# volume-em/empanada-napari

Measured on AMD Instinct MI355X. Metric: EM tiles/sec (1024^2 fp16), higher is better.
Workload: dtype f16

## Files before the change

### empanada-napari_amd/csrc/conv3x3c64.hip

```cpp
#include "igemm_common.h"

namespace emp {
namespace {

constexpr int C64_TH = 8, C64_TW = 16;
constexpr int C64_IH = C64_TH + 2, C64_IW = C64_TW + 2;
constexpr int C64_NPIX = C64_IH * C64_IW;
constexpr int C64_NPC = (C64_NPIX + 7) / 8;
constexpr int C64_SLOT = (C64_NPC + 1) * 1024;
constexpr int C64_NDMA = 3;

struct C64Params {
  const half_t* in;
  const half_t* wgt;
  const float* bias;
  half_t* out;
  const half_t* zero;
  int N, H, W, in_ld, out_ld, act;
  int tiles_x, tiles_y, tiles;
};

template <int ACT>
__global__ void __launch_bounds__(512, 1) conv3x3_c64_kernel(const C64Params p) {
  extern __shared__ __attribute__((aligned(1024))) char lds[];
  const int tid = threadIdx.x, lane = tid & 63;
  const int wave = __builtin_amdgcn_readfirstlane(tid >> 6);
  const int pg = wave >> 1, ch = wave & 1;
  const int fr = lane & 15, fq = lane >> 4;

  const int xcd = blockIdx.x & 7, jx = blockIdx.x >> 3, nx = gridDim.x >> 3;
  auto tile_of = [&](int it) { return (it * 8 + xcd) * nx + jx; };
  int my_tiles = 0;
  while (tile_of(my_tiles) < p.tiles) ++my_tiles;

  f16x8 wreg[2][9][2];
#pragma unroll
  for (int c = 0; c < 2; ++c) {
    const half_t* wr = p.wgt + (size_t)(ch * 32 + perm32(c * 16 + fr)) * (9 * 64) + fq * 8;
#pragma unroll
    for (int t = 0; t < 9; ++t)
#pragma unroll
      for (int kk = 0; kk < 2; ++kk) wreg[c][t][kk] = *reinterpret_cast<const f16x8*>(wr + t * 64 + kk * 32);
  }
  float bv[8];
  {
    const int co = ch * 32 + fq * 8;
#pragma unroll
    for (int r = 0; r < 8; ++r) bv[r] = p.bias ? p.bias[co + r] : 0.f;
  }
  asm volatile("s_waitcnt vmcnt(0)" ::: "memory");

  auto stage = [&](int it, int slot) {
    const bool valid = it < my_tiles;
    int n = 0, y0 = 0, x0 = 0;
    if (valid) {
      const int tile = tile_of(it);
      const int tx = tile % p.tiles_x, r = tile / p.tiles_x;
      const int ty = r % p.tiles_y;
      n = r / p.tiles_y;
      y0 = ty * C64_TH;
      x0 = tx * C64_TW;
    }
    char* hb = lds + slot * C64_SLOT;
#pragma unroll
    for (int k = 0; k < C64_NDMA; ++k) {
      const int piece = wave + 8 * k;
      const int hp = piece * 8 + (lane >> 3);
      const int hy = hp / C64_IW, hx = hp - hy * C64_IW;
      const int iy = y0 + hy - 1, ix = x0 + hx - 1;
      const bool ok = valid && wave + 8 * k < C64_NPC && hp < C64_NPIX && (unsigned)iy < (unsigned)p.H &&
                      (unsigned)ix < (unsigned)p.W;
      const half_t* src = ok ? p.in + (((size_t)n * p.H + iy) * p.W + ix) * p.in_ld + (((lane & 7) ^ (hp & 7)) << 3)
                             : p.zero;
      lds_dma16(src, hb + piece * 1024);
    }
  };

  stage(0, 0);
  stage(1, 1);
  asm volatile("s_waitcnt vmcnt(3)" ::: "memory");
  lds_barrier();

  int slot = 0;
  for (int it = 0; it < my_tiles; ++it) {
    stage(it + 2, slot == 0 ? 2 : slot - 1);
    const char* hb = lds + slot * C64_SLOT;
    f32x4 acc[2][2];
#pragma unroll
    for (int c = 0; c < 2; ++c)
#pragma unroll
      for (int t = 0; t < 2; ++t) acc[c][t] = f32x4{0.f, 0.f, 0.f, 0.f};
#pragma unroll
    for (int tap = 0; tap < 9; ++tap) {
      const int dy = tap / 3, dx = tap - dy * 3;
#pragma unroll
      for (int kk = 0; kk < 2; ++kk) {
        f16x8 pf[2];
#pragma unroll
        for (int t = 0; t < 2; ++t) {
          const int hp = (2 * pg + t + dy) * C64_IW + fr + dx;
          pf[t] = *reinterpret_cast<const f16x8*>(hb + hp * 128 + (((kk * 4 + fq) ^ (hp & 7)) << 4));
        }
#pragma unroll
        for (int c = 0; c < 2; ++c)
#pragma unroll
          for (int t = 0; t < 2; ++t)
            acc[c][t] = __builtin_amdgcn_mfma_f32_16x16x32_f16(wreg[c][tap][kk], pf[t], acc[c][t], 0, 0, 0);
      }
    }
    asm volatile("s_waitcnt vmcnt(3)" ::: "memory");
    {
      const int tile = tile_of(it);
      const int tx = tile % p.tiles_x, r = tile / p.tiles_x;
      const int ty = r % p.tiles_y, n = r / p.tiles_y;
      const int ox = tx * C64_TW + fr;
#pragma unroll
      for (int t = 0; t < 2; ++t) {
        const int oy = ty * C64_TH + 2 * pg + t;
        f16x8 o;
#pragma unroll
        for (int r4 = 0; r4 < 4; ++r4) {
          o[r4] = (half_t)conv_act<ACT>(acc[0][t][r4] + bv[r4]);
          o[4 + r4] = (half_t)conv_act<ACT>(acc[1][t][r4] + bv[4 + r4]);
        }
        if (oy < p.H && ox < p.W)
          *reinterpret_cast<f16x8*>(p.out + (((size_t)n * p.H + oy) * p.W + ox) * p.out_ld + ch * 32 + fq * 8) = o;
      }
    }
    lds_barrier();
    slot = slot == 2 ? 0 : slot + 1;
  }
  asm volatile("s_waitcnt vmcnt(0)" ::: "memory");
}

constexpr int C128_NDMA = 6;
constexpr int C128_SLOT = 8 * C128_NDMA * 1024;

template <int ACT>
__global__ void __launch_bounds__(512, 1) conv3x3_c128_kernel(const C64Params p) {
  extern __shared__ __attribute__((aligned(1024))) char lds[];
  const int tid = threadIdx.x, lane = tid & 63;
  const int wave = __builtin_amdgcn_readfirstlane(tid >> 6);
  const int fr = lane & 15, fq = lane >> 4;
  const int xcd = blockIdx.x & 7, jx = blockIdx.x >> 3, nx = gridDim.x >> 3;
  auto tile_of = [&](int it) { return (it * 8 + xcd) * nx + jx; };
  int my_tiles = 0;
  while (tile_of(my_tiles) < p.tiles) ++my_tiles;

  f16x8 wreg[9][4];
  {
    const half_t* wr = p.wgt + (size_t)(16 * wave + fr) * (9 * 128) + fq * 8;
#pragma unroll
    for (int t = 0; t < 9; ++t)
#pragma unroll
      for (int kk = 0; kk < 4; ++kk) wreg[t][kk] = *reinterpret_cast<const f16x8*>(wr + t * 128 + kk * 32);
  }
  float bv[4];
#pragma unroll
  for (int r = 0; r < 4; ++r) bv[r] = p.bias ? p.bias[16 * wave + fq * 4 + r] : 0.f;
  asm volatile("s_waitcnt vmcnt(0)" ::: "memory");

  auto tile_xy = [&](int it, int& n, int& y0, int& x0) {
    const int tile = tile_of(it);
    const int tx = tile % p.tiles_x, r = tile / p.tiles_x;
    const int ty = r % p.tiles_y;
    n = r / p.tiles_y;
    y0 = ty * C64_TH;
    x0 = tx * C64_TW;
  };
  auto stage = [&](int it, int slot) {
    const bool valid = it < my_tiles;
    int n = 0, y0 = 0, x0 = 0;
    if (valid) tile_xy(it, n, y0, x0);
    char* hb = lds + slot * C128_SLOT;
#pragma unroll
    for (int k = 0; k < C128_NDMA; ++k) {
      const int piece = wave + 8 * k;
      const int hp = piece * 4 + (lane >> 4);
      const int hy = hp / C64_IW, hx = hp - hy * C64_IW;
      const int iy = y0 + hy - 1, ix = x0 + hx - 1;
      const bool ok = valid && hp < C64_NPIX && (unsigned)iy < (unsigned)p.H && (unsigned)ix < (unsigned)p.W;
      const half_t* src = ok ? p.in + (((size_t)n * p.H + iy) * p.W + ix) * p.in_ld + (((lane & 15) ^ (hp & 15)) << 3)
                             : p.zero;
      lds_dma16(src, hb + piece * 1024);
    }
  };

  stage(0, 0);
  stage(1, 1);
  asm volatile("s_waitcnt vmcnt(6)" ::: "memory");
  lds_barrier();

  int slot = 0;
  for (int it = 0; it < my_tiles; ++it) {
    stage(it + 2, slot == 0 ? 2 : slot - 1);
    char* hb = lds + slot * C128_SLOT;
    f32x4 acc[8];
#pragma unroll
    for (int y = 0; y < 8; ++y) acc[y] = f32x4{0.f, 0.f, 0.f, 0.f};
    int frv = fr;
    asm volatile("" : "+v"(frv));
#pragma unroll
    for (int g = 0; g < 3 * C64_IH; ++g) {
      const int r = g / 3, dx = g - r * 3;
      const int hp = r * C64_IW + frv + dx;
      f16x8 pf[4];
#pragma unroll
      for (int kk = 0; kk < 4; ++kk)
        pf[kk] = *reinterpret_cast<const f16x8*>(hb + hp * 256 + (((kk * 4 + fq) ^ (hp & 15)) << 4));
#pragma unroll
      for (int kk = 0; kk < 4; ++kk)
#pragma unroll
        for (int dy = 0; dy < 3; ++dy) {
          const int y = r - dy;
          if (y >= 0 && y < 8) acc[y] = __builtin_amdgcn_mfma_f32_16x16x32_f16(wreg[dy * 3 + dx][kk], pf[kk], acc[y], 0, 0, 0);
        }
      __builtin_amdgcn_sched_barrier(0);
    }
    asm volatile("s_waitcnt vmcnt(6)" ::: "memory");
    lds_barrier();
#pragma unroll
    for (int y = 0; y < 8; ++y) {
      const int px = y * 16 + fr;
      typedef _Float16 f16x4 __attribute__((ext_vector_type(4)));
      f16x4 o;
#pragma unroll
      for (int r4 = 0; r4 < 4; ++r4) o[r4] = (half_t)conv_act<ACT>(acc[y][r4] + bv[r4]);
      const int chunk = 2 * wave + (fq >> 1);
      *reinterpret_cast<f16x4*>(hb + px * 256 + ((chunk ^ (px & 15)) << 4) + (fq & 1) * 8) = o;
    }
    lds_barrier();
    {
      int n, y0, x0;
      tile_xy(it, n, y0, x0);
#pragma unroll
      for (int k = 0; k < 4; ++k) {
        const int q = k * 512 + tid;
        const int px = q >> 4, c = q & 15;
        const int oy = y0 + (px >> 4), ox = x0 + (px & 15);
        const f16x8 v = *reinterpret_cast<const f16x8*>(hb + px * 256 + ((c ^ (px & 15)) << 4));
        if (oy < p.H && ox < p.W)
          *reinterpret_cast<f16x8*>(p.out + (((size_t)n * p.H + oy) * p.W + ox) * p.out_ld + c * 8) = v;
      }
    }
    lds_barrier();
    slot = slot == 2 ? 0 : slot + 1;
  }
  asm volatile("s_waitcnt vmcnt(0)" ::: "memory");
}

}

bool conv3x3_c64_supported(const ConvParams& p) {
  return ((p.Cin == 64 && p.Cout == 64) || (p.Cin == 128 && p.Cout == 128)) && p.KH == 3 && p.KW == 3 && p.stride == 1 && p.pad == 1 && p.dil == 1 &&
         p.res == nullptr && p.bias_n == nullptr && p.ps_cout == 0 && p.in2 == nullptr && p.out2 == nullptr;
}

int launch_conv3x3_c64(const ConvParams& q, hipStream_t stream) {
  EMP_REQUIRE(conv3x3_c64_supported(q), "conv3x3_c64: unsupported shape");
  C64Params p{};
  p.in = q.in; p.wgt = q.wgt; p.bias = q.bias; p.out = q.out; p.zero = q.zero;
  p.N = q.N; p.H = q.H; p.W = q.W; p.in_ld = q.in_ld; p.out_ld = q.out_ld; p.act = q.act;
  p.tiles_x = cdiv(q.W, C64_TW);
  p.tiles_y = cdiv(q.H, C64_TH);
  p.tiles = q.N * p.tiles_x * p.tiles_y;
  int grid = 256;
  while (grid > 8 && grid > p.tiles) grid -= 8;
  auto go = [&](auto kern) -> int { return launch_dyn(kern, grid, 512, 3 * C64_SLOT, stream, p); };
  auto go128 = [&](auto kern) -> int { return launch_dyn(kern, grid, 512, 3 * C128_SLOT, stream, p); };
  if (q.Cin == 128) {
    if (q.act == 1) return go128(&conv3x3_c128_kernel<1>);
    if (q.act == 2) return go128(&conv3x3_c128_kernel<2>);
    return go128(&conv3x3_c128_kernel<0>);
  }
  if (q.act == 1) return go(&conv3x3_c64_kernel<1>);
  if (q.act == 2) return go(&conv3x3_c64_kernel<2>);
  return go(&conv3x3_c64_kernel<0>);
}

}
```

Measured before the change: 1372.

## Overlap c128 conv output writeback with next tile's MFMA loop and split fragment loads

Measured after the change: 1376 (median of 6 runs). About the same (+0.3%).

```diff
diff --git a/empanada-napari_amd/csrc/conv3x3c64.hip b/empanada-napari_amd/csrc/conv3x3c64.hip
--- a/empanada-napari_amd/csrc/conv3x3c64.hip
+++ b/empanada-napari_amd/csrc/conv3x3c64.hip
@@ -135,6 +135,11 @@
 
 constexpr int C128_NDMA = 6;
 constexpr int C128_SLOT = 8 * C128_NDMA * 1024;
+
+__device__ __forceinline__ void halo_dma16(const void* src, const void* dst) {
+  const unsigned l = (unsigned)(size_t)(const __attribute__((address_space(3))) void*)dst;
+  asm volatile("s_mov_b32 m0, %1\n\ts_nop 0\n\tglobal_load_lds_dwordx4 %0, off" ::"v"(src), "s"(l) : "memory");
+}
 
 template <int ACT>
 __global__ void __launch_bounds__(512, 1) conv3x3_c128_kernel(const C64Params p) {
@@ -182,8 +187,17 @@
       const bool ok = valid && hp < C64_NPIX && (unsigned)iy < (unsigned)p.H && (unsigned)ix < (unsigned)p.W;
       const half_t* src = ok ? p.in + (((size_t)n * p.H + iy) * p.W + ix) * p.in_ld + (((lane & 15) ^ (hp & 15)) << 3)
                              : p.zero;
-      lds_dma16(src, hb + piece * 1024);
-    }
+      halo_dma16(src, hb + piece * 1024);
+    }
+  };
+
+  const int rb_row = tid >> 8, rb_col = (tid >> 4) & 15;
+  const int rb_lds = (tid >> 4) * 256 + (((tid & 15) ^ rb_col) << 4);
+  const unsigned rb_off = ((unsigned)(rb_row * p.W + rb_col) * p.out_ld + (tid & 15) * 8) * 2;
+  auto rb_read = [&](const char* ob, int k) { return *reinterpret_cast<const f16x8*>(ob + k * 8192 + rb_lds); };
+  auto rb_store = [&](int k, int n, int y0, int x0, const f16x8& v) {
+    char* base = reinterpret_cast<char*>(p.out) + (((size_t)n * p.H + y0 + 2 * k) * p.W + x0) * p.out_ld * 2;
+    if (y0 + 2 * k + rb_row < p.H && x0 + rb_col < p.W) *reinterpret_cast<f16x8*>(base + rb_off) = v;
   };
 
   stage(0, 0);
@@ -193,32 +207,54 @@
 
   int slot = 0;
   for (int it = 0; it < my_tiles; ++it) {
-    stage(it + 2, slot == 0 ? 2 : slot - 1);
+    const int pslot = slot == 0 ? 2 : slot - 1;
     char* hb = lds + slot * C128_SLOT;
+    const char* ob = lds + pslot * C128_SLOT;
+    int pn = 0, py0 = p.H, px0 = 0;
+    if (it > 0) tile_xy(it - 1, pn, py0, px0);
     f32x4 acc[8];
 #pragma unroll
     for (int y = 0; y < 8; ++y) acc[y] = f32x4{0.f, 0.f, 0.f, 0.f};
     int frv = fr;
     asm volatile("" : "+v"(frv));
-#pragma unroll
-    for (int g = 0; g < 3 * C64_IH; ++g) {
-      const int r = g / 3, dx = g - r * 3;
+    auto frag = [&](int h, f16x8 (&pf)[2]) {
+      const int g = h >> 1, r = g / 3, dx = g - r * 3;
       const int hp = r * C64_IW + frv + dx;
-      f16x8 pf[4];
-#pragma unroll
-      for (int kk = 0; kk < 4; ++kk)
-        pf[kk] = *reinterpret_cast<const f16x8*>(hb + hp * 256 + (((kk * 4 + fq) ^ (hp & 15)) << 4));
-#pragma unroll
-      for (int kk = 0; kk < 4; ++kk)
+#pragma unroll
+      for (int j = 0; j < 2; ++j)
+        pf[j] = *reinterpret_cast<const f16x8*>(hb + hp * 256 + ((((h & 1) * 8 + j * 4 + fq) ^ (hp & 15)) << 4));
+    };
+    auto mac = [&](int h, const f16x8 (&pf)[2]) {
+      const int g = h >> 1, r = g / 3, dx = g - r * 3;
+#pragma unroll
+      for (int j = 0; j < 2; ++j)
 #pragma unroll
         for (int dy = 0; dy < 3; ++dy) {
           const int y = r - dy;
-          if (y >= 0 && y < 8) acc[y] = __builtin_amdgcn_mfma_f32_16x16x32_f16(wreg[dy * 3 + dx][kk], pf[kk], acc[y], 0, 0, 0);
+          if (y >= 0 && y < 8)
+            acc[y] = __builtin_amdgcn_mfma_f32_16x16x32_f16(wreg[dy * 3 + dx][(h & 1) * 2 + j], pf[j], acc[y], 0, 0, 0);
         }
+    };
+    f16x8 pa[2], pb[2], rb;
+    frag(0, pa);
+#pragma unroll
+    for (int g = 0; g < 3 * C64_IH; ++g) {
+      frag(2 * g + 1, pb);
+      if (g < 4) rb = rb_read(ob, g);
       __builtin_amdgcn_sched_barrier(0);
-    }
-    asm volatile("s_waitcnt vmcnt(6)" ::: "memory");
+      mac(2 * g, pa);
+      __builtin_amdgcn_sched_barrier(0);
+      if (g + 1 < 3 * C64_IH) frag(2 * g + 2, pa);
+      __builtin_amdgcn_sched_barrier(0);
+      mac(2 * g + 1, pb);
+      __builtin_amdgcn_sched_barrier(0);
+      if (g < 4) {
+        rb_store(g, pn, py0, px0, rb);
+        __builtin_amdgcn_sched_barrier(0);
+      }
+    }
     lds_barrier();
+    stage(it + 2, pslot);
 #pragma unroll
     for (int y = 0; y < 8; ++y) {
       const int px = y * 16 + fr;
@@ -229,22 +265,16 @@
       const int chunk = 2 * wave + (fq >> 1);
       *reinterpret_cast<f16x4*>(hb + px * 256 + ((chunk ^ (px & 15)) << 4) + (fq & 1) * 8) = o;
     }
-    lds_barrier();
-    {
-      int n, y0, x0;
-      tile_xy(it, n, y0, x0);
-#pragma unroll
-      for (int k = 0; k < 4; ++k) {
-        const int q = k * 512 + tid;
-        const int px = q >> 4, c = q & 15;
-        const int oy = y0 + (px >> 4), ox = x0 + (px & 15);
-        const f16x8 v = *reinterpret_cast<const f16x8*>(hb + px * 256 + ((c ^ (px & 15)) << 4));
-        if (oy < p.H && ox < p.W)
-          *reinterpret_cast<f16x8*>(p.out + (((size_t)n * p.H + oy) * p.W + ox) * p.out_ld + c * 8) = v;
-      }
-    }
+    asm volatile("s_waitcnt vmcnt(6)" ::: "memory");
     lds_barrier();
     slot = slot == 2 ? 0 : slot + 1;
+  }
+  if (my_tiles > 0) {
+    const char* ob = lds + (slot == 0 ? 2 : slot - 1) * C128_SLOT;
+    int n, y0, x0;
+    tile_xy(my_tiles - 1, n, y0, x0);
+#pragma unroll
+    for (int k = 0; k < 4; ++k) rb_store(k, n, y0, x0, rb_read(ob, k));
   }
   asm volatile("s_waitcnt vmcnt(0)" ::: "memory");
 }
```
